# learnedsystems/RMI

Hardware: AMD Instinct MI355X
Metric: keys/s trained (200M uint64, linear,linear 1048576 leaves) (higher is better)
Workload: dtype f64

## Files before the change

### rmi_amd/csrc/rmi_hip.hip

```cpp
#include <hip/hip_runtime.h>

#include <algorithm>
#include <atomic>
#include <cstdarg>
#include <cstdio>
#include <cstdlib>
#include <cstring>
#include <cmath>
#include <functional>
#include <mutex>
#include <string>
#include <thread>
#include <vector>

#include "../../include/rmi_hip.h"
#include "rmi_kernels.hip.h"
#include "rmi_stream.hip.h"
#include "rmi_sigma.hip.h"
#include "rmi_lanes.hip.h"
#include "rmi_regs.hip.h"
#include "rmi_scan_launch.h"
#include "rmi_lookup_launch.h"
#include "rmi_root_host.h"
#include "rmi_route.h"
// ... 40 lines not shown
  rmi_route::Route last_route;
  bool tail_armed = false;
  std::function<int()> tail_fn;
  std::function<int(unsigned int)> regs_listed_fn;
  std::function<void()> refinalize_fn;
  unsigned int* d_tickets = nullptr;
  int peer_fuse_n = 0;
  unsigned char* peer_fuse_tab[7] = {};
  bool rows_pushed = false;
  hipEvent_t ev_stage[2] = {nullptr, nullptr};
  hipEvent_t ev[10] = {};
  int profile_level = 0;
  DevState* h_state_dev = nullptr;
  double* d_lntab = nullptr;
  double* d_regtab = nullptr;
  unsigned long long* d_regprof = nullptr;
  std::vector<rmi_hip_ctx*> many_views;
  void* d_bnext = nullptr; uint64_t bnext_cap = 0;
  unsigned char* d_tile_slow = nullptr; uint64_t tile_slow_cap = 0;
  unsigned int* d_slow_list = nullptr; uint64_t slow_cap = 0;
  int n_cu = 256;
  void* d_gaps = nullptr;
  unsigned int* d_tile_list = nullptr; uint64_t tile_list_cap = 0;
  bool lean_derived = false;
  unsigned long long lean_last_target = ~0ull, lean_leaf_lo = 0;
  uint64_t edge_first = 0, edge_last = 0, edge_epoch = 0, edgef_epoch = 0; double edge_first_f = 0.0, edge_last_f = 0.0;
  GiantLeaf* d_giant = nullptr; uint64_t giant_cap = 0;
  bool giant_armed = false;
  static constexpr uint64_t GIANT_EARLY_MAX = 256;
  unsigned long long* h_giant = nullptr;
// ... 84 lines not shown
  return RMI_OK;
}

extern "C" {

int rmi_hip_abi_version(void) { return RMI_HIP_ABI_VERSION; }
int rmi_hip_last_pipeline(rmi_hip_ctx* c) { return !c ? RMI_ERR_BAD_ARG : c->last_route.pipeline; }
int rmi_hip_last_route_info(rmi_hip_ctx* c, rmi_hip_route_info* out) {
  if (!c || !out || !c->last_L || !c->h_state) return RMI_ERR_BAD_ARG;
  const rmi_route::Route& r = c->last_route;
  const DevState& st = *c->h_state;
  std::memset(out, 0, sizeof *out);
  out->pipeline = r.pipeline; out->regs = r.regs;
  out->search = r.search; out->verify = r.verify; out->cubic_margin = r.cubic_margin; out->sigma = r.sigma;
  out->scan_mono = r.scan_mono; out->long_leaves = r.long_leaves; out->giants = r.giants;
  out->regs_listed = st.regs_listed; out->scan_listed = st.scan_listed; out->long_count = st.long_count; out->giant_count = st.giant_count;
  out->flag_count = st.flag_count; out->merged_count = st.merged_count; out->seg_count = st.seg_count; out->regs_dups = st.regs_dups;
  return RMI_OK;
}

int rmi_hip_device_count(void) {
  int n = 0;
  if (hipGetDeviceCount(&n) != hipSuccess) return 0;
  return n;
}

const char* rmi_hip_strerror(int code) {
  switch (code) {
    case RMI_OK: return "ok";
    case RMI_ERR_UNKNOWN_MODEL: return "unknown model type (train/mod.rs:53)";
// ... 82 lines not shown
  if (hipStreamCreateWithFlags(&c->own_stream, hipStreamNonBlocking) != hipSuccess) { rmi_hip_destroy(c); return RMI_ERR_HIP; }
  c->stream = c->own_stream;
  if (hipMalloc(&c->d_state, sizeof(DevState)) != hipSuccess) { rmi_hip_destroy(c); return RMI_ERR_HIP; }
  if (hipHostMalloc((void**)&c->h_state, sizeof(DevState) * RMI_STREAM_MAX_CHUNKS, hipHostMallocDefault) != hipSuccess ||
      hipHostGetDevicePointer((void**)&c->h_state_dev, c->h_state, 0) != hipSuccess) { rmi_hip_destroy(c); return RMI_ERR_HIP; }
  if (hipHostMalloc((void**)&c->h_sentinel, 64, hipHostMallocDefault) != hipSuccess) { rmi_hip_destroy(c); return RMI_ERR_HIP; }
  for (auto& e : c->ev) if (hipEventCreate(&e) != hipSuccess) { rmi_hip_destroy(c); return RMI_ERR_HIP; }
  c->profile_level = 0;
  c->knobs = rmi_route::read_knobs();
  { int cu = 0; if (hipDeviceGetAttribute(&cu, hipDeviceAttributeMultiprocessorCount, device_id) == hipSuccess && cu > 0) c->n_cu = cu; }
  if (hipMalloc(&c->d_lntab, sizeof(double) * (3 * LN_TMAX + 2 * (LS_SAMPLES + 1))) != hipSuccess) { rmi_hip_destroy(c); return RMI_ERR_HIP; }
  hipLaunchKernelGGL(k_lane_table, dim3((LN_TMAX + 255) / 256), dim3(256), 0, c->stream, c->d_lntab, LN_TMAX);
  if (hipMalloc(&c->d_regtab, sizeof(double) * 4 * RG_TMAX) != hipSuccess) { rmi_hip_destroy(c); return RMI_ERR_HIP; }
  if (RG_PROF) { if (hipMalloc(&c->d_regprof, 128) != hipSuccess || hipMemset(c->d_regprof, 0, 128) != hipSuccess) { rmi_hip_destroy(c); return RMI_ERR_HIP; } }
  hipLaunchKernelGGL(k_regs_table, dim3((RG_TMAX + 255) / 256), dim3(256), 0, c->stream, c->d_regtab, RG_TMAX);
  if (hipGetLastError() != hipSuccess || hipStreamSynchronize(c->stream) != hipSuccess) { rmi_hip_destroy(c); return RMI_ERR_HIP; }
  *out = c;
  return RMI_OK;
}

static void free_outputs(rmi_hip_ctx* c) {
  (void)hipFree(c->d_leaf_start); (void)hipFree(c->d_params); (void)hipFree(c->d_maxerr); (void)hipFree(c->d_run);
  (void)hipFree(c->d_err); (void)hipFree(c->d_count); (void)hipFree(c->d_rows); (void)hipFree(c->d_tilemin);
  (void)hipFree(c->d_partials); c->d_partials = nullptr;
  (void)hipFree(c->d_tickets); c->d_tickets = nullptr;
  release(c->d_long, c->long_cap); release(c->d_cube, c->cube_cap); release(c->d_flist, c->flist_cap); release(c->d_tile_list, c->tile_list_cap);
  release(c->d_bkeys, c->bkeys_cap); release(c->d_recs, c->recs_bytes); release(c->d_segs, c->segs_cap);
  if (c->d_flist_cnt) { (void)hipFree(c->d_flist_cnt); c->d_flist_cnt = nullptr; }
  if (c->d_gaps) { (void)hipFree(c->d_gaps); c->d_gaps = nullptr; }
  c->d_leaf_start = nullptr; c->d_params = nullptr; c->d_maxerr = nullptr; c->d_run = nullptr;
// ... 6 lines not shown
  if (!c) return;
  for (rmi_hip_ctx* v : c->many_views) rmi_hip_destroy(v);
  c->many_views.clear();
  for (rmi_hip_index* ix : c->indexes) index_release(ix);
  c->indexes.clear();
  if (c->upload_thread.joinable()) c->upload_thread.join();
  (void)hipSetDevice(c->device);
  if (c->stream) (void)hipStreamSynchronize(c->stream);
  free_multi(c);
  free_outputs(c);
  if (c->d_table) (void)hipFree(c->d_table);
  if (c->d_keys_owned) (void)hipFree(c->d_keys_owned);
  if (c->d_state) (void)hipFree(c->d_state);
  if (c->d_lntab) (void)hipFree(c->d_lntab);
  if (c->d_regtab) (void)hipFree(c->d_regtab);
  if (c->d_regprof) {
    unsigned long long h[16] = {};
    if (hipMemcpy(h, c->d_regprof, 128, hipMemcpyDeviceToHost) == hipSuccess)
      std::fprintf(stderr, "k_leaf_regs cycles (sum over waves and trainings): fit %llu, epilogue+tail %llu, hand-over %llu, error pass %llu, finalize %llu; (unused %llu) hand-over requests %llu, (unused %llu), finalize stores %llu, finalize up to the shuffles' end %llu; RG_PROF 2, inside the fit: panel requests %llu, stash %llu, arithmetic %llu, constants + landed %llu, wait for the panel %llu\n", h[0], h[1], h[2], h[3], h[4], h[5], h[6], h[7], h[8], h[9], h[5], h[7], h[8], h[9], h[11]);
    (void)hipFree(c->d_regprof);
  }
  release(c->d_slow_list, c->slow_cap); release(c->d_tile_slow, c->tile_slow_cap); release(c->d_bnext, c->bnext_cap); release(c->d_giant, c->giant_cap);
  if (c->h_state) (void)hipHostFree(c->h_state);
  if (c->h_sentinel) (void)hipHostFree(c->h_sentinel);
  for (int b = 0; b < 2; b++) { if (c->h_stage[b]) (void)hipHostFree(c->h_stage[b]); if (c->ev_stage[b]) (void)hipEventDestroy(c->ev_stage[b]); }
  if (c->copy_stream) (void)hipStreamDestroy(c->copy_stream);
  if (c->h_giant) (void)hipHostFree(c->h_giant);
  if (c->ev_giant) (void)hipEventDestroy(c->ev_giant);
  for (auto& e : c->ev) if (e) (void)hipEventDestroy(e);
  if (c->own_stream) (void)hipStreamDestroy(c->own_stream);
// ... 653 lines not shown

static inline uint64_t agg_records(uint64_t leaves) { const uint64_t w = (leaves + 63) / 64, m = (uint64_t)SCAN_MAX_WAVES + SCAN_GAP_BLOCKS; return w > m ? w : m; }
static inline uint64_t lane_slices(uint64_t leaves) { return (agg_records(leaves) + LF_SLICE - 1) / LF_SLICE; }
static int ensure_outputs(rmi_hip_ctx* c, uint64_t L, int ppl) {
  if (L <= c->cap_leaves && ppl <= c->cap_ppl) return RMI_OK;
  free_outputs(c);
  HIPCHK(c, hipMalloc(&c->d_leaf_start, (L + 1) * 8));
  HIPCHK(c, hipMalloc(&c->d_params, L * ppl * 8));
  HIPCHK(c, hipMalloc(&c->d_maxerr, L * 8));
  HIPCHK(c, hipMalloc(&c->d_run, L * 8));
  HIPCHK(c, hipMalloc(&c->d_err, L * 8));
  HIPCHK(c, hipMalloc(&c->d_count, L * 8));
  HIPCHK(c, hipMalloc(&c->d_rows, L * (ppl * 8 + 8)));
  HIPCHK(c, hipMalloc(&c->d_tilemin, ((L + 1 + FILL_TILE - 1) / FILL_TILE + 1) * 8));
  HIPCHK(c, hipMalloc(&c->d_partials, sizeof(StatsPartial) * (agg_records(L) + SG_REGIONS + 2 * FL_BLOCKS + 1 + lane_slices(L) + 1)));
  HIPCHK(c, hipMalloc(&c->d_tickets, 64));
  c->cap_leaves = L; c->cap_ppl = ppl;
  return RMI_OK;
}

static void host_cubes(double* v, uint64_t n) {
  unsigned nt = std::thread::hardware_concurrency();
  nt = nt < 1 ? 1 : (nt > 16 ? 16 : nt);
  if (n < 65536) nt = 1;
  auto work = [v](uint64_t a, uint64_t b) { for (uint64_t i = a; i < b; i++) v[i] = std::pow(v[i], 3.0); };
  if (nt == 1) { work(0, n); return; }
  std::vector<std::thread> th;
  const uint64_t per = (n + nt - 1) / nt;
  for (unsigned t = 0; t < nt; t++) {
    const uint64_t a = (uint64_t)t * per, b = a + per < n ? a + per : n;
    if (a < b) th.emplace_back(work, a, b);
// ... 90 lines not shown
    }
    if (r.giants_early) (void)launch_giant_list(c, a, fl);
    hipLaunchKernelGGL((k_list<K, LEAF>), dim3(128 * SG_REGIONS), dim3(64), 0, a.s, a.keys, a.sp, a.leaf_start, c->d_state, a.params, fl, sgp, a.maxerr, a.run,
                       dgiant, hmin, !r.giants_early);
    mk();
    hipLaunchKernelGGL((k_list_tail<K>), dim3(2048), dim3(64), 0, a.s, a.keys, a.sp, a.leaf_start, c->d_state, a.params, fl, c->d_segs, a.maxerr, a.run,
                       r.fused ? (const StatsPartial*)part : (const StatsPartial*)nullptr, (unsigned int)nrec, part + nrec);
    mk();
    if (r.fused)
      hipLaunchKernelGGL((k_finalize_listed<K>), dim3(FL_BLOCKS), dim3(FL_THREADS), 0, a.s, a.keys, a.sp, a.L, a.leaf_start, c->d_state, a.params, a.maxerr, a.run, a.err,
                         a.count, a.rows, fl, part + nrec, (unsigned int)SG_REGIONS, part + nrec + SG_REGIONS, c->d_flist_cnt + 2 * SG_REGIONS, c->d_state, hcopy,
                         (const GiantLeaf*)nullptr, hmin);
  };
  if (r.optimistic) {
    const unsigned int nsl = (unsigned int)((nrec + LF_SLICE - 1) / LF_SLICE);
    hipLaunchKernelGGL(k_lane_reduce, dim3(nsl), dim3(LF_SLICE), 0, a.s, (const StatsPartial*)part, (unsigned int)nrec, part + nrec + SG_REGIONS + 2 * FL_BLOCKS + 1,
                       c->d_tickets, fl, c->d_state, hcopy);
    a.mark(); a.mark();
    c->tail_armed = true;
    c->giant_early = r.giants_early;
    c->tail_fn = [tail]() -> int { tail([]() {}); return RMI_OK; };
  } else tail(a.mark);
}

template <typename K>
static int launch_regs(rmi_hip_ctx* c, const rmi_route::Route& r, const RootP& rp, Launch<K>& a, const SgList& fl, const PeerRows& peers) {
  const uint64_t wb = (a.L_own + 63) / 64;
  if (const int grc = grow(c, c->d_slow_list, c->slow_cap, wb, 4)) return grc;
  if (const int grc = grow(c, c->d_tile_slow, c->tile_slow_cap, wb, 1)) return grc;
  if (const int grc = grow(c, c->d_bnext, c->bnext_cap, wb, 64 * 16)) return grc;
  HIPCHK(c, hipGetLastError());
  const unsigned int lmin = lanes_long_min(c);
// ... 9 lines not shown
  else if constexpr (sizeof(K) == 4) regs(std::integral_constant<int, 2>{});
  a.mark();
  auto listed = [=](unsigned int grid_l) {
    hipLaunchKernelGGL((k_leaf_lanes_listed<K>), dim3(grid_l), dim3(64), 0, a.s, c->d_slow_list, c->d_tickets + 1, a.keys, a.sp, a.leaf_start, c->d_state, a.params,
                       c->d_lntab, fl, lmin, a.maxerr, a.run, a.L, a.err, a.count, a.rows, part, rp, peers);
  };
  if (r.listed_late) {
    const unsigned int wb_l = (unsigned int)wb;
    c->regs_listed_fn = [=](unsigned int groups) -> int {
      listed(groups < wb_l ? (groups > 0u ? groups : 1u) : wb_l);
      hipLaunchKernelGGL(k_lane_reduce, dim3((wb_l + LF_SLICE - 1) / LF_SLICE), dim3(LF_SLICE), 0, a.s, (const StatsPartial*)part, wb_l,
                         part + wb + SG_REGIONS + 2 * FL_BLOCKS + 1, c->d_tickets, fl, c->d_state, c->h_state_dev);
      return RMI_OK;
    };
  } else listed(wb < 512 ? (unsigned int)wb : 512u);
  auto finalize = [&](auto vroot, double scale) {
    hipLaunchKernelGGL((k_regs_finalize<K, decltype(vroot)::value>), dim3((unsigned)((wb * 64 + 255) / 256)), dim3(256), 0, a.s, a.keys, a.sp, a.L, a.leaf_start, c->d_state,
                       (const unsigned int*)(c->d_tickets + 1), a.params, (const unsigned long long*)a.maxerr, (const K*)bnext, (const K*)bprev,
                       (const unsigned char*)c->d_tile_slow, (unsigned int)wb, a.err, a.count, a.rows, part, peers, rp, scale, r.listed_late);
  };
  if (r.cubic_margin) finalize(std::integral_constant<int, K_CUBIC>{}, c->knobs.cubic_margin_scale);
  else finalize(std::integral_constant<int, -1>{}, 1.0);
  HIPCHK(c, hipGetLastError());
  return RMI_OK;
}

template <int ROOT, typename K>
static int launch_leaf_lanes(rmi_hip_ctx* c, const rmi_route::Route& r, const RootP& rp, Launch<K>& a) {
  hipStream_t s = a.s;
  const uint64_t L_own = a.L_own, wb = (L_own + 63) / 64;
  if (const int lrc = ensure_lists(c, a.n_it, L_own)) return lrc;
  if constexpr (ROOT == K_LINEAR || ROOT == K_RADIX || ROOT == K_CUBIC) {
    if (r.search) {
      const uint64_t sb = (L_own + (uint64_t)LS_BLOCK * LS_ILP - 1) / ((uint64_t)LS_BLOCK * LS_ILP);
      double* smp = c->d_lntab + 3 * LN_TMAX;
      LaneInit li; std::memset(&li, 0, sizeof li);
      if (r.init_folded) {
        li.st = c->d_state; li.init = a.init; li.leaf_start = a.a_leaf_start; li.L_own = L_own; li.sentinel = (unsigned long long)a.sp.it_hi;
        li.list_cnt = c->d_flist_cnt; li.n_list_cnt = 2 * SG_REGIONS + 8; li.tickets = c->d_tickets; li.n_tickets = 3;
      }
      hipLaunchKernelGGL((k_leaf_samples<ROOT, K>), dim3((LS_SAMPLES + 256) / 256), dim3(256), 0, s, a.keys, a.sp, rp, smp, li);
      hipLaunchKernelGGL((k_leaf_search<ROOT, K, LS_ILP>), dim3((unsigned)sb), dim3(LS_BLOCK), 0, s, a.keys, a.sp, rp, a.leaf_start, c->d_state, (const double*)smp);
    }
  }
  if (!r.init_folded) HIPCHK(c, hipMemsetAsync(c->d_tickets, 0, 12, s));
  if (!r.search) {
    launch_bounds<ROOT, K>(s, a.keys, a.n_it, a.sp, rp, a.leaf_start, c->d_state);
    launch_fill(s, a.a_leaf_start, L_own + 1, c->d_tilemin);
  }
  HIPCHK(c, a.mark.begin());
  const SgList fl = flist_of(c);
  if (r.giants) { if (const int grc = arm_giants(c, a)) return grc; }
  const PeerRows peers = peer_rows(c, r);
  auto lanes = [&](auto fused, auto vroot) {
// ... 556 lines not shown
```

### rmi_amd/csrc/rmi_lanes.hip.h

```cpp
#pragma once
#include <type_traits>

#include "rmi_device.hip.h"
#include "rmi_kernels.hip.h"
#include "rmi_stream.hip.h"
#include "rmi_sigma.hip.h"

#ifndef RMI_LN_NT_FIT
#define RMI_LN_NT_FIT 0
#endif
#ifndef RMI_LN_NT_ERR
#define RMI_LN_NT_ERR 1
#endif
#ifndef RMI_LN_WPE
#define RMI_LN_WPE 2
#endif
#ifndef RMI_LN_NBUF
#define RMI_LN_NBUF 2
#endif

namespace rmi {

template <typename K> struct LnGeom {
  static constexpr int KPL = 16 / (int)sizeof(K);
// ... 26 lines not shown

template <int ROOT, typename K>
__device__ __forceinline__ double ls_root_value(const RootP& r, K k) {
  if constexpr (ROOT == K_RADIX) {
    const uint64_t v = KeyTraits<K>::as_uint(k) << (r.prefix & 63u);
    return ldexp(KeyTraits<uint64_t>::as_float(v), -(int)((64u - r.bits) & 63u));
  } else return root_eval_f<ROOT>(r, KeyTraits<K>::as_float(k));
}

constexpr int LS_SAMPLES = 1024;
__device__ __forceinline__ uint64_t ls_sample_index(uint64_t A, uint64_t Bn, int t) {
  const uint64_t stride = (Bn - A - 1) / (uint64_t)LS_SAMPLES > 0 ? (Bn - A - 1) / (uint64_t)LS_SAMPLES : 1;
  const uint64_t i = A + (uint64_t)t * stride;
  return (t >= LS_SAMPLES || i >= Bn) ? Bn - 1 : i;
}
struct LaneInit {
  DevState* st; DevState init;
  unsigned long long* leaf_start; uint64_t L_own; unsigned long long sentinel;
  unsigned long long* list_cnt; int n_list_cnt;
  unsigned int* tickets; unsigned int n_tickets;
};
template <int ROOT, typename K>
__global__ void __launch_bounds__(256) k_leaf_samples(const K* __restrict__ keys, Span sp, RootP r, double* __restrict__ smp, LaneInit li) {
  const int t = blockIdx.x * 256 + threadIdx.x;
  if (li.st != nullptr && blockIdx.x == gridDim.x - 1) {
    for (int q = threadIdx.x; q < li.n_list_cnt; q += 256) li.list_cnt[q] = 0ull;
    for (unsigned int q = threadIdx.x; q < li.n_tickets; q += 256u) li.tickets[q] = 0u;
    if (threadIdx.x == 0) { *li.st = li.init; li.leaf_start[li.L_own] = li.sentinel; }
  }
  if (t > LS_SAMPLES || !(sp.it_hi > sp.it_lo)) return;
  const K k = keys[ls_sample_index(sp.it_lo, sp.it_hi, t)];
  bool oob;
  smp[t] = root_target_f<ROOT, K>(r, (double)(r.L - 1), k, oob);
  smp[LS_SAMPLES + 1 + t] = ls_root_value<ROOT, K>(r, k);
}

template <int ROOT, typename K, int ILP>
__global__ void __launch_bounds__(LS_BLOCK) k_leaf_search(const K* __restrict__ keys, Span sp, RootP r,
                                                          unsigned long long* __restrict__ leaf_start,
                                                          DevState* __restrict__ st, const double* __restrict__ smp) {
  typedef typename LnBits<K>::type BT;
  typedef BT vec_t __attribute__((ext_vector_type(2), aligned(sizeof(K))));
// ... 560 lines not shown
  if (!s_last) return;
  StatsPartial b{0ull, 0ull, 0ull, 0.0, 0.0};
  for (unsigned int t = threadIdx.x; t < gridDim.x; t += LF_SLICE) lf_combine(b, lf_load(slices + t));
  lf_block_reduce(b, &s_w);
  unsigned long long fc = threadIdx.x < (unsigned int)SG_REGIONS ? fl.cnt[threadIdx.x] : 0ull;
#pragma unroll
  for (int d = 32; d > 0; d >>= 1) fc += shfl_down_u64(fc, d);
  if (threadIdx.x == 0) {
    *ticket = 0u;
    st->max_err = b.mx; st->max_err_idx = b.mi; st->sum_n_err = b.sum; st->sum_l2 = b.l2; st->sum_log2 = b.lg;
    st->flag_count = fc; st->merged_count = 0; st->pending = fc;
    *host_copy = *st;
  }
}

constexpr int FL_BLOCKS = 1;
constexpr int FL_THREADS = 256;
template <typename K>
__global__ void __launch_bounds__(FL_THREADS) k_finalize_listed(const K* __restrict__ keys, Span sp, uint64_t L,
                                                         const unsigned long long* __restrict__ leaf_start,
                                                         const DevState* __restrict__ st, double* __restrict__ params,
                                                         const unsigned long long* __restrict__ leaf_maxerr,
                                                         const unsigned long long* __restrict__ leaf_run,
                                                         unsigned long long* __restrict__ leaf_err,
                                                         unsigned long long* __restrict__ leaf_count,
                                                         unsigned char* __restrict__ rows, SgList fl,
                                                         const StatsPartial* __restrict__ wave_partials, unsigned int nwave,
                                                         StatsPartial* __restrict__ out, unsigned long long* __restrict__ ticket,
                                                         DevState* __restrict__ stw, DevState* __restrict__ host_copy,
                                                         const GiantLeaf* __restrict__ flat, unsigned long long host_min) {
// ... 100 lines not shown
```

### rmi_amd/csrc/rmi_regs.hip.h

```cpp
#pragma once
#include <type_traits>

#include "rmi_lanes.hip.h"

namespace rmi {

#ifndef RG_STASH_N
#define RG_STASH_N 192
#endif
constexpr int RG_ROW = 16;
constexpr int RG_RING = 4;
constexpr int RG_PANEL_B = 64 * RG_ROW * 8;
constexpr int RG_STASH = RG_STASH_N;
#ifndef RG_STASH2_N
#define RG_STASH2_N 160
#endif
constexpr int RG_STASH2 = RG_STASH2_N;
constexpr int RG_MAXPTS = RG_STASH_N + 48;
constexpr int RG_FARPTS = 1008;
constexpr int RG_NBLK = RG_MAXPTS / RG_ROW;
constexpr int RG_SBLK = RG_STASH / RG_ROW;
static_assert(RG_NBLK - RG_SBLK <= RG_RING - 1, "the tail of a group must still be in the ring when its fit ends");
static_assert(RG_FARPTS + 16 <= 1024, "the step table (RG_TMAX) covers the walk");

// ... 633 lines not shown
    have = true;
    done_tile = tile;
    tile = tile2;
    tile2 = (unsigned int)__builtin_amdgcn_readfirstlane((int)tile3);
  }
  if (RG_PROF && prof != nullptr && lane == 0) {
#pragma unroll
    for (int i = 0; i < 12; i++) atomicAdd(prof + i, pf[i]);
  }
}

__device__ __forceinline__ uint64_t rg_readlane_u64(uint64_t v, int src) {
  const unsigned int lo = (unsigned int)__builtin_amdgcn_readlane((int)(unsigned int)v, src), hi = (unsigned int)__builtin_amdgcn_readlane((int)(unsigned int)(v >> 32), src);
  return ((uint64_t)hi << 32) | lo;
}
template <typename K, int VROOT = -1>
__global__ void __launch_bounds__(256) k_regs_finalize(const K* __restrict__ keys, Span sp, uint64_t L,
                                                       const unsigned long long* __restrict__ leaf_start, DevState* st, const unsigned int* __restrict__ slow_count,
                                                       double* __restrict__ params, const unsigned long long* __restrict__ leaf_maxerr,
                                                       const K* __restrict__ bnext, const K* __restrict__ bprev,
                                                       const unsigned char* __restrict__ tile_slow, unsigned int ntiles,
                                                       unsigned long long* __restrict__ leaf_err, unsigned long long* __restrict__ leaf_count,
                                                       unsigned char* __restrict__ rows, StatsPartial* __restrict__ partials, PeerRows peers, RootP vr,
                                                       double margin_scale,
                                                       bool listed_behind) {
  const uint64_t jl = (uint64_t)blockIdx.x * 256 + threadIdx.x;
  const unsigned int tile = (unsigned int)(jl >> 6);
  if (jl == 0) st->regs_listed = *slow_count;
  if (tile >= ntiles) return;
  const uint64_t j = sp.leaf_lo + jl;
  if constexpr (VROOT == K_CUBIC) {
    bool ok = true;
    uint64_t vs = 0, ve = 0;
    if (j < sp.leaf_hi) {
      const uint64_t s = leaf_start[j], e = leaf_start[j + 1];
      vs = s; ve = e;
      if (s < e) {
        auto val = [&](K k) -> double {
          const double x = KeyTraits<K>::as_float(k);
          const double v1 = __builtin_fma(vr.p0, x, vr.p1), v2 = __builtin_fma(v1, x, vr.p2), v3 = __builtin_fma(v2, x, vr.p3);
          return v3;
        };
        const uint64_t nl = sp.leaf_hi - sp.leaf_lo;
// ... 14 lines not shown
    const unsigned int Lm1 = (unsigned int)(vr.L - 1);
    while (um) {
      const int src = __builtin_ctzll(um);
      um &= um - 1ull;
      const uint64_t us = rg_readlane_u64(vs, src), ue = rg_readlane_u64(ve, src);
      const unsigned int uj = (unsigned int)(sp.leaf_lo + (jl & ~63ull) + (uint64_t)src);
      for (uint64_t i = us + (threadIdx.x & 63); i < ue; i += 64) {
        const unsigned int rt = sg_cvt_u32(root_eval_f<K_CUBIC>(vr, KeyTraits<K>::as_float(keys[i])));
        if (rt > Lm1) vflags |= EF_ROOT_OOB;
        if ((rt < Lm1 ? rt : Lm1) != uj) vflags |= EF_NON_MONOTONE;
      }
    }
    if (vflags) atomicOr(&st->err_flags, vflags);
  }
  if (tile_slow[tile] != 0) {
    if (listed_behind && (threadIdx.x & 63) == 0) partials[tile] = StatsPartial{0ull, 0ull, 0ull, 0.0, 0.0};
    return;
  }
  unsigned long long st_mx = 0, st_mi = 0, st_sum = 0;
  double st_l2 = 0.0, st_lg = 0.0;
  unsigned long long me = 0ull;
  uint64_t fs = 0, fe = 0;
  double fa = 0.0, fb = 0.0;
  if (j < sp.leaf_hi) { me = leaf_maxerr[j]; fs = leaf_start[j]; fe = leaf_start[j + 1]; fa = params[2 * j]; fb = params[2 * j + 1]; }
  {
    unsigned long long um = __ballot((me >> 63) != 0ull);
    const unsigned int n32 = (unsigned int)sp.n;
    const int ln = (int)(threadIdx.x & 63);
    while (um) {
      const int src = __builtin_ctzll(um);
      um &= um - 1ull;
// ... 5 lines not shown
        const double f = __builtin_fma(ub, KeyTraits<K>::as_float(keys[i]), ua);
        em = max(em, sg_absdiff(min(sg_cvt_u32(f), n32), (unsigned int)i));
      }
      em = rg_wave_max(em);
      if (ln == src) me = (unsigned long long)em;
    }
  }
  if (j < sp.leaf_hi) {
    const uint64_t s = fs, e = fe;
    double pp[2] = {fa, fb};
    const K k_next = e < sp.n ? bnext[jl] : KeyTraits<K>::max_value();
    const K k_prev = s > 0 ? bprev[jl] : KeyTraits<K>::zero_value();
    uint64_t final_err, cnt_j;
    finalize_one_pre<K_LINEAR, K>(j, s, e, sp, L, keys, pp, me, 0ull, st->last_target, k_next, k_prev, final_err, cnt_j);
    if (!(s < e)) { params[2 * j] = pp[0]; params[2 * j + 1] = pp[1]; }
    leaf_err[j] = final_err;
    leaf_count[j] = cnt_j;
    double* rp = reinterpret_cast<double*>(rows + j * 24);
    rp[0] = pp[0]; rp[1] = pp[1];
    *reinterpret_cast<unsigned long long*>(rows + j * 24 + 16) = final_err;
    for (int p = 0; p < peers.n; p++) {
      double* pr = reinterpret_cast<double*>(peers.tab[p] + j * 24);
      pr[0] = pp[0]; pr[1] = pp[1];
      *reinterpret_cast<unsigned long long*>(peers.tab[p] + j * 24 + 16) = final_err;
    }
    st_mx = final_err; st_mi = j;
    st_sum = cnt_j * final_err;
    const double v = (double)st_sum;
    st_l2 = (v * v) / (double)sp.n;
    st_lg = (double)cnt_j * log2((double)(2 * final_err + 2));
  }
#pragma unroll
  for (int d = 32; d > 0; d >>= 1) {
    const unsigned long long omx = shfl_down_u64(st_mx, d), omi = shfl_down_u64(st_mi, d);
    if (omx > st_mx || (omx == st_mx && omi > st_mi)) { st_mx = omx; st_mi = omi; }
    st_sum += shfl_down_u64(st_sum, d);
    st_l2 += __shfl_down(st_l2, d);
    st_lg += __shfl_down(st_lg, d);
  }
  if ((threadIdx.x & 63) == 0) partials[tile] = StatsPartial{st_mx, st_mi, st_sum, st_l2, st_lg};
}

template <typename K>
__global__ void __launch_bounds__(64) __attribute__((amdgpu_waves_per_eu(RMI_LN_WPE, RMI_LN_WPE))) k_leaf_lanes_listed(const unsigned int* __restrict__ slow_list,
                                                   const unsigned int* __restrict__ slow_count, const K* __restrict__ keys, Span sp,
                                                   const unsigned long long* __restrict__ leaf_start,
                                                   DevState* __restrict__ st, double* __restrict__ params,
                                                   const double* __restrict__ rtab, SgList fl, unsigned int long_min,
                                                   unsigned long long* __restrict__ leaf_maxerr,
                                                   unsigned long long* __restrict__ leaf_run, uint64_t L,
                                                   unsigned long long* __restrict__ leaf_err,
                                                   unsigned long long* __restrict__ leaf_count,
                                                   unsigned char* __restrict__ rows, StatsPartial* __restrict__ partials, RootP vr,
                                                   PeerRows peers) {
  __shared__ typename LnBits<K>::type panel[64 * LnGeom<K>::STRIDE];
// ... 8 lines not shown
```

### rmi_amd/csrc/rmi_route.h

```cpp
#pragma once

#include <algorithm>
#include <cstdint>
#include <cstdlib>
#include <functional>

#include "../../include/rmi_hip.h"

namespace rmi_route {

constexpr uint64_t IDX32_LIMIT = (1ull << 32) - (1ull << 16);
constexpr uint64_t SIGMA_MIN_LEAF = 32;
constexpr uint64_t SCAN_SKEW_LISTED = 512;

struct Knobs {
  int pipeline = 3;
  bool lanes_search = true;
  bool opt_tail = true;
  uint64_t host_min = 262144;
  bool host_min_set = false;
  bool regs = true;
  bool regs_forced = false;
  int regs_u32 = 2;
  unsigned int regs_grid = 0;
  unsigned int regs_max_avg = 208;
  unsigned int regs_long_max_avg = 640;
  bool regs_backoff = true;
  bool cubic_margin = true;
  double cubic_margin_scale = 1.0;
  bool lean = true;
  unsigned int scan_waves = 0;
  uint64_t fit_threads = 131072;
  int fit_min_chunk = 64;
  unsigned int long_min = 4096;
};

inline Knobs read_knobs() {
  Knobs k;
  auto env = [](const char* name) -> const char* { const char* v = std::getenv(name); return v && *v ? v : nullptr; };
  if (const char* v = env("RMI_HIP_PIPELINE")) k.pipeline = std::atoi(v) >= 3 ? 3 : 2;
  if (const char* v = env("RMI_HIP_LANES_SEARCH")) k.lanes_search = std::atoi(v) != 0;
  if (const char* v = env("RMI_HIP_OPT_TAIL")) k.opt_tail = std::atoi(v) != 0;
  if (const char* v = env("RMI_HIP_HOST_MIN")) { k.host_min = std::strtoull(v, nullptr, 10); k.host_min_set = true; }
  if (const char* v = env("RMI_HIP_REGS")) { k.regs = std::atoi(v) != 0; k.regs_forced = k.regs; }
  if (const char* v = env("RMI_HIP_REGS_U32")) k.regs_u32 = std::atoi(v);
  if (const char* v = env("RMI_HIP_REGS_GRID")) k.regs_grid = (unsigned int)std::atoi(v);
  if (const char* v = env("RMI_HIP_REGS_MAX_AVG")) k.regs_max_avg = (unsigned int)std::atoi(v);
  if (const char* v = env("RMI_HIP_REGS_LONG_MAX_AVG")) k.regs_long_max_avg = (unsigned int)std::atoi(v);
  if (const char* v = env("RMI_HIP_REGS_BACKOFF")) k.regs_backoff = std::atoi(v) != 0;
  if (const char* v = env("RMI_HIP_CUBIC_MARGIN")) k.cubic_margin = std::atoi(v) != 0;
  if (const char* v = env("RMI_HIP_CUBIC_MARGIN_SCALE")) k.cubic_margin_scale = std::atof(v);
  if (const char* v = env("RMI_HIP_LEAN")) k.lean = std::atoi(v) != 0;
  if (const char* v = env("RMI_HIP_SCAN_WAVES")) k.scan_waves = (unsigned int)std::atoi(v);
  if (const char* v = env("RMI_HIP_FIT_THREADS")) k.fit_threads = std::strtoull(v, nullptr, 10);
  if (const char* v = env("RMI_HIP_FIT_MIN_CHUNK")) k.fit_min_chunk = std::atoi(v);
  if (const char* v = env("RMI_HIP_LONG_MIN")) { const long l = std::atol(v); if (l >= 64) k.long_min = (unsigned int)l; }
  return k;
// ... 16 lines not shown

struct Route {
  int pipeline = 2;
  bool sigma = false;
  bool search = false;
  bool init_folded = false;
  bool fused = false;
  bool optimistic = false;
  bool listed_late = false;
  bool peers = false;
  bool giants = false, giants_early = false;
  int regs = -1;
  unsigned int regs_grid = 0;
  bool verify = false;
  bool cubic_margin = false;
  bool scan_mono = false, lean = false, long_leaves = false;
  unsigned int listed_hint = ~0u;
  bool lanes() const { return pipeline >= 3; }
  bool init_arrays() const { return pipeline != 5 && !init_folded; }
};

inline Route plan_route(const Knobs& k, const RouteIn& in) {
  Route r;
  const bool idx32 = in.n < IDX32_LIMIT, u32 = in.key_type == RMI_KEY_U32;
  const bool linear_leaf = in.leaf_kind == RMI_MODEL_LINEAR;
  const bool linear_root = in.root_kind == RMI_MODEL_LINEAR || in.root_kind == RMI_MODEL_ROBUST_LINEAR || in.root_kind == RMI_MODEL_LINEAR_SPLINE;
  const bool radix_root = in.root_kind == RMI_MODEL_RADIX || in.root_kind == RMI_MODEL_BRADIX, cubic_root = in.root_kind == RMI_MODEL_CUBIC;
  const uint64_t L = in.L_own;
  const bool scan = k.pipeline >= 3 && in.leaf_kind == RMI_MODEL_LINEAR_SPLINE && idx32;
  r.sigma = linear_leaf && in.fit_mode != 0 && !in.sigma_hinted && idx32 && in.n_it >= SIGMA_MIN_LEAF * L && in.n_it >= 4096;
// ... 20 lines not shown
  }
  r.pipeline = 3;
  const uint64_t wb = (L + 63) / 64, resident = 4ull * (uint64_t)in.n_cu;
  const bool regs_long = in.n_it > (uint64_t)k.regs_max_avg * L;
  const unsigned int cap = k.regs_long_max_avg > k.regs_max_avg ? k.regs_long_max_avg : k.regs_max_avg;
  bool regs = r.fused && k.regs && !in.regs_off && in.n_it <= (uint64_t)cap * L && (!u32 || k.regs_u32);
  if (!regs_long && !k.regs_forced && k.regs_grid == 0 && wb > resident && 2 * wb <= 5 * resident) regs = false;
  if (cubic_root && linear_leaf && r.search && regs && k.cubic_margin) r.cubic_margin = in.cubic_increasing();
  r.verify = cubic_root && linear_leaf && r.search && !r.cubic_margin;
  if (regs && !r.verify) {
    r.pipeline = 4;
    const bool w2 = u32 && k.regs_u32 >= 2;
    r.regs = w2 ? 2 : regs_long ? 1 : 0;
    const uint64_t grid = k.regs_grid ? k.regs_grid : (w2 ? 8ull : 4ull) * (uint64_t)in.n_cu;
    r.regs_grid = (unsigned int)(grid > wb ? wb : grid);
  }
  return r;
}

struct RouteKey { uint64_t epoch; uint64_t L_own; int fit_mode; };
struct TrainCounts { uint64_t scan_listed, flag_count, merged_count; unsigned int regs_listed; };
struct RouteMemory {
  uint64_t hint_epoch = 0, hint_L[8] = {};
  int hint_n = 0, hint_mode = -1;
  uint64_t regs_off_epoch = 0, regs_off_L[8] = {};
  int regs_off_n = 0;
  uint64_t scan_hint_epoch = 0, scan_hint_L = 0; unsigned int scan_hint_n = ~0u;
  uint64_t scan_skew_epoch = ~0ull, scan_skew_L = 0;

  void lookup(const RouteKey& key, RouteIn* in) const {
// ... 24 lines not shown
```

### rmi_amd/train.py

```python
from __future__ import annotations

import ctypes as C
import re
import threading
import time
from dataclasses import dataclass, field

import numpy as np

from . import _lib

KEY_U64, KEY_U32, KEY_F64 = 0, 1, 2
_DTYPES = {np.dtype(np.uint64): KEY_U64, np.dtype(np.uint32): KEY_U32, np.dtype(np.float64): KEY_F64}

MODEL_NAMES = ["linear", "linear_spline", "cubic", "radix", "robust_linear", "loglinear", "normal",
               "lognormal", "radix8", "radix18", "radix22", "radix26", "radix28", "bradix", "histogram"]


class RMIError(RuntimeError):

    def __init__(self, code: int, detail: str = ""):
        lib = _lib.load()
        msg = lib.rmi_hip_strerror(code).decode()
        super().__init__(f"rmi_hip error {code}: {msg}" + (f" [{detail}]" if detail else ""))
# ... 316 lines not shown
            device_ns=int(res.device_ns), kernel_ns=tuple(res.kernel_ns), long_leaves=int(res.long_leaves),
            split_idx=int(res.split_idx), split_target=int(res.split_target),
            shard_leaf_lo=int(res.shard_leaf_lo), shard_leaves=int(res.shard_leaves),
            partial={"max_error": int(res.model_max_error), "max_error_idx": int(res.model_max_error_idx),
                     "sum_n_err": int(res.sum_n_err), "sum_l2": float(res.sum_l2), "sum_log2": float(res.sum_log2)},
            fit_mode_used=int(res.fit_mode_used), exact_leaves=int(res.exact_leaves), merged_leaves=int(res.merged_leaves), guard_leaves=int(res.guard_leaves),
            generation=int(res.generation), pipeline=int(self._lib.rmi_hip_last_pipeline(self._h)), _trainer=self)

    def last_route(self):
        fn = getattr(self._lib, "rmi_hip_last_route_info", None)
        info = _lib.RouteInfo()
        with self._ctx_lock:
            if fn is None or self._h is None or fn(self._h, C.byref(info)) != 0:
                return None
        flags = ("search", "verify", "cubic_margin", "sigma", "scan_mono", "long_leaves", "giants")
        return {n: (bool(getattr(info, n)) if n in flags else int(getattr(info, n))) for n, _ in _lib.RouteInfo._fields_ if not n.startswith("_")}

    def train_many(self, configs, in_flight: int = 4):
        self.wait_keys()
        n = len(configs)
        cfg = (_lib.TrainConfig * max(n, 1))()
        kinds, keep = [], []
        for i, (root, leaf, L) in enumerate(configs):
            lk = leaf if isinstance(leaf, int) else MODEL_NAMES.index(leaf)
            kinds.append(lk)
            cfg[i].root = root._c()
            cfg[i].leaf_kind = lk
            cfg[i].num_leaves = int(L)
            if root.is_radix_table:
                if root.table is None:
                    raise ValueError("a radix-table root needs its hint table (Model.table)")
# ... 142 lines not shown
```

Measured before the change: 427.0 billion.

## Fuse lane stats reduction into regs finalize via last-block tickets

Removes the separate k_lane_reduce launch by having k_regs_finalize blocks count arrivals per slice with atomics. The last block of each slice reduces the slice, and the last slice publishes the global stats to device and host state. It also replaces the per-leaf log2 with a precomputed table for small errors, swaps the final four shuffle rounds for DPP row shifts, and in lean mode skips the per-leaf err/count writes. The cost is extra atomics and a tail serialisation in the last blocks, plus more complex ticket reset logic.

```diff
diff --git a/rmi_amd/csrc/rmi_hip.hip b/rmi_amd/csrc/rmi_hip.hip
--- a/rmi_amd/csrc/rmi_hip.hip
+++ b/rmi_amd/csrc/rmi_hip.hip
@@ -78,6 +78,7 @@
   DevState* h_state_dev = nullptr;
   double* d_lntab = nullptr;
   double* d_regtab = nullptr;
+  double* d_l2tab = nullptr;
   unsigned long long* d_regprof = nullptr;
   std::vector<rmi_hip_ctx*> many_views;
   void* d_bnext = nullptr; uint64_t bnext_cap = 0;
@@ -192,6 +193,7 @@
   out->pipeline = r.pipeline; out->regs = r.regs;
   out->search = r.search; out->verify = r.verify; out->cubic_margin = r.cubic_margin; out->sigma = r.sigma;
   out->scan_mono = r.scan_mono; out->long_leaves = r.long_leaves; out->giants = r.giants;
+  out->_pad = (r.tail_fused ? 1 : 0) | (r.lean ? 2 : 0);
   out->regs_listed = st.regs_listed; out->scan_listed = st.scan_listed; out->long_count = st.long_count; out->giant_count = st.giant_count;
   out->flag_count = st.flag_count; out->merged_count = st.merged_count; out->seg_count = st.seg_count; out->regs_dups = st.regs_dups;
   return RMI_OK;
@@ -304,6 +306,8 @@
   if (hipMalloc(&c->d_regtab, sizeof(double) * 4 * RG_TMAX) != hipSuccess) { rmi_hip_destroy(c); return RMI_ERR_HIP; }
   if (RG_PROF) { if (hipMalloc(&c->d_regprof, 128) != hipSuccess || hipMemset(c->d_regprof, 0, 128) != hipSuccess) { rmi_hip_destroy(c); return RMI_ERR_HIP; } }
   hipLaunchKernelGGL(k_regs_table, dim3((RG_TMAX + 255) / 256), dim3(256), 0, c->stream, c->d_regtab, RG_TMAX);
+  if (hipMalloc(&c->d_l2tab, sizeof(double) * RG_L2TAB) != hipSuccess) { rmi_hip_destroy(c); return RMI_ERR_HIP; }
+  hipLaunchKernelGGL(k_regs_log2_table, dim3((RG_L2TAB + 255) / 256), dim3(256), 0, c->stream, c->d_l2tab, RG_L2TAB);
   if (hipGetLastError() != hipSuccess || hipStreamSynchronize(c->stream) != hipSuccess) { rmi_hip_destroy(c); return RMI_ERR_HIP; }
   *out = c;
   return RMI_OK;
@@ -340,6 +344,7 @@
   if (c->d_state) (void)hipFree(c->d_state);
   if (c->d_lntab) (void)hipFree(c->d_lntab);
   if (c->d_regtab) (void)hipFree(c->d_regtab);
+  if (c->d_l2tab) (void)hipFree(c->d_l2tab);
   if (c->d_regprof) {
     unsigned long long h[16] = {};
     if (hipMemcpy(h, c->d_regprof, 128, hipMemcpyDeviceToHost) == hipSuccess)
@@ -1023,7 +1028,7 @@
   HIPCHK(c, hipMalloc(&c->d_rows, L * (ppl * 8 + 8)));
   HIPCHK(c, hipMalloc(&c->d_tilemin, ((L + 1 + FILL_TILE - 1) / FILL_TILE + 1) * 8));
   HIPCHK(c, hipMalloc(&c->d_partials, sizeof(StatsPartial) * (agg_records(L) + SG_REGIONS + 2 * FL_BLOCKS + 1 + lane_slices(L) + 1)));
-  HIPCHK(c, hipMalloc(&c->d_tickets, 64));
+  HIPCHK(c, hipMalloc(&c->d_tickets, 4 * lf_ticket_words(lane_slices(L))));
   c->cap_leaves = L; c->cap_ppl = ppl;
   return RMI_OK;
 }
@@ -1144,8 +1149,9 @@
   };
   if (r.optimistic) {
     const unsigned int nsl = (unsigned int)((nrec + LF_SLICE - 1) / LF_SLICE);
-    hipLaunchKernelGGL(k_lane_reduce, dim3(nsl), dim3(LF_SLICE), 0, a.s, (const StatsPartial*)part, (unsigned int)nrec, part + nrec + SG_REGIONS + 2 * FL_BLOCKS + 1,
-                       c->d_tickets, fl, c->d_state, hcopy);
+    if (!r.tail_fused)
+      hipLaunchKernelGGL(k_lane_reduce, dim3(nsl), dim3(LF_SLICE), 0, a.s, (const StatsPartial*)part, (unsigned int)nrec, part + nrec + SG_REGIONS + 2 * FL_BLOCKS + 1,
+                         c->d_tickets, fl, c->d_state, hcopy);
     a.mark(); a.mark();
     c->tail_armed = true;
     c->giant_early = r.giants_early;
@@ -1185,13 +1191,19 @@
       return RMI_OK;
     };
   } else listed(wb < 512 ? (unsigned int)wb : 512u);
-  auto finalize = [&](auto vroot, double scale) {
-    hipLaunchKernelGGL((k_regs_finalize<K, decltype(vroot)::value>), dim3((unsigned)((wb * 64 + 255) / 256)), dim3(256), 0, a.s, a.keys, a.sp, a.L, a.leaf_start, c->d_state,
-                       (const unsigned int*)(c->d_tickets + 1), a.params, (const unsigned long long*)a.maxerr, (const K*)bnext, (const K*)bprev,
-                       (const unsigned char*)c->d_tile_slow, (unsigned int)wb, a.err, a.count, a.rows, part, peers, rp, scale, r.listed_late);
+  LaneTail lt; std::memset(&lt, 0, sizeof lt);
+  lt.slices = part + wb + SG_REGIONS + 2 * FL_BLOCKS + 1; lt.tickets = c->d_tickets; lt.fl = fl; lt.host_copy = c->h_state_dev;
+  auto finalize = [&](auto vroot, auto fused, double scale) {
+    hipLaunchKernelGGL((k_regs_finalize<K, decltype(vroot)::value, decltype(fused)::value>), dim3((unsigned)((wb * 64 + 255) / 256)), dim3(256), 0, a.s, a.keys, a.sp, a.L,
+                       a.leaf_start, c->d_state, (const unsigned int*)(c->d_tickets + 1), a.params, (const unsigned long long*)a.maxerr, (const K*)bnext, (const K*)bprev,
+                       (const unsigned char*)c->d_tile_slow, (unsigned int)wb, r.lean ? nullptr : a.err, r.lean ? nullptr : a.count, a.rows, part, peers, rp, scale, r.listed_late,
+                       lt, (const double*)c->d_l2tab);
   };
-  if (r.cubic_margin) finalize(std::integral_constant<int, K_CUBIC>{}, c->knobs.cubic_margin_scale);
-  else finalize(std::integral_constant<int, -1>{}, 1.0);
+  auto finalize_root = [&](auto fused) {
+    if (r.cubic_margin) finalize(std::integral_constant<int, K_CUBIC>{}, fused, c->knobs.cubic_margin_scale);
+    else finalize(std::integral_constant<int, -1>{}, fused, 1.0);
+  };
+  if (r.tail_fused) finalize_root(std::true_type{}); else finalize_root(std::false_type{});
   HIPCHK(c, hipGetLastError());
   return RMI_OK;
 }
@@ -1209,6 +1221,7 @@
       if (r.init_folded) {
         li.st = c->d_state; li.init = a.init; li.leaf_start = a.a_leaf_start; li.L_own = L_own; li.sentinel = (unsigned long long)a.sp.it_hi;
         li.list_cnt = c->d_flist_cnt; li.n_list_cnt = 2 * SG_REGIONS + 8; li.tickets = c->d_tickets; li.n_tickets = 3;
+        li.n_slice_cnt = r.tail_fused ? (unsigned int)((wb + LF_SLICE - 1) / LF_SLICE) : 0u;
       }
       hipLaunchKernelGGL((k_leaf_samples<ROOT, K>), dim3((LS_SAMPLES + 256) / 256), dim3(256), 0, s, a.keys, a.sp, rp, smp, li);
       hipLaunchKernelGGL((k_leaf_search<ROOT, K, LS_ILP>), dim3((unsigned)sb), dim3(LS_BLOCK), 0, s, a.keys, a.sp, rp, a.leaf_start, c->d_state, (const double*)smp);
diff --git a/rmi_amd/csrc/rmi_lanes.hip.h b/rmi_amd/csrc/rmi_lanes.hip.h
--- a/rmi_amd/csrc/rmi_lanes.hip.h
+++ b/rmi_amd/csrc/rmi_lanes.hip.h
@@ -64,11 +64,13 @@
   const uint64_t i = A + (uint64_t)t * stride;
   return (t >= LS_SAMPLES || i >= Bn) ? Bn - 1 : i;
 }
+constexpr unsigned int LF_CNT_BASE = 16, LF_CNT_STRIDE = 16;
 struct LaneInit {
   DevState* st; DevState init;
   unsigned long long* leaf_start; uint64_t L_own; unsigned long long sentinel;
   unsigned long long* list_cnt; int n_list_cnt;
   unsigned int* tickets; unsigned int n_tickets;
+  unsigned int n_slice_cnt;
 };
 template <int ROOT, typename K>
 __global__ void __launch_bounds__(256) k_leaf_samples(const K* __restrict__ keys, Span sp, RootP r, double* __restrict__ smp, LaneInit li) {
@@ -76,6 +78,7 @@
   if (li.st != nullptr && blockIdx.x == gridDim.x - 1) {
     for (int q = threadIdx.x; q < li.n_list_cnt; q += 256) li.list_cnt[q] = 0ull;
     for (unsigned int q = threadIdx.x; q < li.n_tickets; q += 256u) li.tickets[q] = 0u;
+    for (unsigned int q = threadIdx.x; q < li.n_slice_cnt; q += 256u) li.tickets[LF_CNT_BASE + q * LF_CNT_STRIDE] = 0u;
     if (threadIdx.x == 0) { *li.st = li.init; li.leaf_start[li.L_own] = li.sentinel; }
   }
   if (t > LS_SAMPLES || !(sp.it_hi > sp.it_lo)) return;
@@ -666,6 +669,56 @@
   }
 }
 
+static inline uint64_t lf_ticket_words(uint64_t slices) { return LF_CNT_BASE + slices * LF_CNT_STRIDE; }
+struct LaneTail {
+  StatsPartial* slices; unsigned int* tickets; SgList fl; DevState* host_copy;
+};
+template <bool OWN_FLAGS>
+__device__ __forceinline__ void lf_arrive_publish(const StatsPartial* partials, unsigned int nrec, const LaneTail& lt, DevState* st, unsigned int regs_listed) {
+  static_assert(LF_SLICE == 128 && SG_REGIONS == 64, "32 blocks of four records a slice; one hand-over counter per lane");
+  constexpr unsigned int BPS = LF_SLICE / 4;
+  __shared__ StatsPartial s_w;
+  __shared__ bool s_last;
+  const unsigned int slice = blockIdx.x / BPS, nsl = (nrec + LF_SLICE - 1) / LF_SLICE;
+  unsigned int* const cnt = lt.tickets + LF_CNT_BASE + slice * LF_CNT_STRIDE;
+  asm volatile("s_waitcnt vmcnt(0)" ::: "memory");
+  __syncthreads();
+  if (threadIdx.x == 0) {
+    const unsigned int left = gridDim.x - slice * BPS, expect = left < BPS ? left : BPS;
+    s_last = __hip_atomic_fetch_add(cnt, 1u, __ATOMIC_RELAXED, __HIP_MEMORY_SCOPE_AGENT) == expect - 1u;
+  }
+  __syncthreads();
+  if (!s_last) return;
+  const unsigned int q = slice * LF_SLICE + threadIdx.x;
+  StatsPartial a{0ull, 0ull, 0ull, 0.0, 0.0};
+  if (threadIdx.x < LF_SLICE && q < nrec) a = lf_load(partials + q);
+  lf_block_reduce(a, &s_w);
+  if (threadIdx.x == 0) {
+    lf_store(lt.slices + slice, a);
+    __hip_atomic_store(cnt, 0u, __ATOMIC_RELAXED, __HIP_MEMORY_SCOPE_AGENT);
+    s_last = __hip_atomic_fetch_add(lt.tickets, 1u, __ATOMIC_RELAXED, __HIP_MEMORY_SCOPE_AGENT) == nsl - 1u;
+  }
+  __syncthreads();
+  if (!s_last) return;
+  StatsPartial b{0ull, 0ull, 0ull, 0.0, 0.0};
+  if (threadIdx.x < LF_SLICE)
+    for (unsigned int t = threadIdx.x; t < nsl; t += LF_SLICE) lf_combine(b, lf_load(lt.slices + t));
+  lf_block_reduce(b, &s_w);
+  unsigned long long fc = threadIdx.x < (unsigned int)SG_REGIONS ? lt.fl.cnt[threadIdx.x] : 0ull;
+#pragma unroll
+  for (int d = 32; d > 0; d >>= 1) fc += shfl_down_u64(fc, d);
+  if (threadIdx.x == 0) {
+    __hip_atomic_store(lt.tickets, 0u, __ATOMIC_RELAXED, __HIP_MEMORY_SCOPE_AGENT);
+    if constexpr (OWN_FLAGS) {
+      st->err_flags = __hip_atomic_fetch_or((volatile unsigned int*)&st->err_flags, 0u, __ATOMIC_RELAXED, __HIP_MEMORY_SCOPE_AGENT);
+    }
+    st->regs_listed = regs_listed;
+    st->max_err = b.mx; st->max_err_idx = b.mi; st->sum_n_err = b.sum; st->sum_l2 = b.l2; st->sum_log2 = b.lg;
+    st->flag_count = fc; st->merged_count = 0; st->pending = fc;
+    *lt.host_copy = *st;
+  }
+}
+
 constexpr int FL_BLOCKS = 1;
 constexpr int FL_THREADS = 256;
 template <typename K>
diff --git a/rmi_amd/csrc/rmi_regs.hip.h b/rmi_amd/csrc/rmi_regs.hip.h
--- a/rmi_amd/csrc/rmi_regs.hip.h
+++ b/rmi_amd/csrc/rmi_regs.hip.h
@@ -671,8 +671,22 @@
   const unsigned int lo = (unsigned int)__builtin_amdgcn_readlane((int)(unsigned int)v, src), hi = (unsigned int)__builtin_amdgcn_readlane((int)(unsigned int)(v >> 32), src);
   return ((uint64_t)hi << 32) | lo;
 }
-template <typename K, int VROOT = -1>
-__global__ void __launch_bounds__(256) k_regs_finalize(const K* __restrict__ keys, Span sp, uint64_t L,
+constexpr int RG_L2TAB = 4096;
+static __global__ void __launch_bounds__(256) k_regs_log2_table(double* __restrict__ tab, int count) {
+  const int e = blockIdx.x * blockDim.x + threadIdx.x;
+  if (e < count) tab[e] = log2((double)(2ull * (unsigned long long)e + 2ull));
+}
+template <int D> __device__ __forceinline__ unsigned long long rg_row_down_u64(unsigned long long v) {
+  const unsigned int lo = (unsigned int)v, hi = (unsigned int)(v >> 32);
+  const unsigned int ol = (unsigned int)__builtin_amdgcn_update_dpp((int)lo, (int)lo, 0x100 + D, 0xF, 0xF, false);
+  const unsigned int oh = (unsigned int)__builtin_amdgcn_update_dpp((int)hi, (int)hi, 0x100 + D, 0xF, 0xF, false);
+  return ((unsigned long long)oh << 32) | ol;
+}
+template <int D> __device__ __forceinline__ double rg_row_down_f64(double v) {
+  return __longlong_as_double((long long)rg_row_down_u64<D>((unsigned long long)__double_as_longlong(v)));
+}
+template <typename K, int VROOT, bool FUSED>
+__device__ __forceinline__ void regs_finalize_leaves(const K* __restrict__ keys, Span sp, uint64_t L,
                                                        const unsigned long long* __restrict__ leaf_start, DevState* st, const unsigned int* __restrict__ slow_count,
                                                        double* __restrict__ params, const unsigned long long* __restrict__ leaf_maxerr,
                                                        const K* __restrict__ bnext, const K* __restrict__ bprev,
@@ -680,10 +694,10 @@
                                                        unsigned long long* __restrict__ leaf_err, unsigned long long* __restrict__ leaf_count,
                                                        unsigned char* __restrict__ rows, StatsPartial* __restrict__ partials, PeerRows peers, RootP vr,
                                                        double margin_scale,
-                                                       bool listed_behind) {
+                                                       bool listed_behind, const double* __restrict__ l2tab) {
   const uint64_t jl = (uint64_t)blockIdx.x * 256 + threadIdx.x;
   const unsigned int tile = (unsigned int)(jl >> 6);
-  if (jl == 0) st->regs_listed = *slow_count;
+  if (!FUSED && jl == 0) st->regs_listed = *slow_count;
   if (tile >= ntiles) return;
   const uint64_t j = sp.leaf_lo + jl;
   if constexpr (VROOT == K_CUBIC) {
@@ -728,7 +742,10 @@
     if (vflags) atomicOr(&st->err_flags, vflags);
   }
   if (tile_slow[tile] != 0) {
-    if (listed_behind && (threadIdx.x & 63) == 0) partials[tile] = StatsPartial{0ull, 0ull, 0ull, 0.0, 0.0};
+    if (listed_behind && (threadIdx.x & 63) == 0) {
+      const StatsPartial none{0ull, 0ull, 0ull, 0.0, 0.0};
+      if constexpr (FUSED) lf_store(partials + tile, none); else partials[tile] = none;
+    }
     return;
   }
   unsigned long long st_mx = 0, st_mi = 0, st_sum = 0;
@@ -764,8 +781,7 @@
     uint64_t final_err, cnt_j;
     finalize_one_pre<K_LINEAR, K>(j, s, e, sp, L, keys, pp, me, 0ull, st->last_target, k_next, k_prev, final_err, cnt_j);
     if (!(s < e)) { params[2 * j] = pp[0]; params[2 * j + 1] = pp[1]; }
-    leaf_err[j] = final_err;
-    leaf_count[j] = cnt_j;
+    if (!FUSED || leaf_err != nullptr) { leaf_err[j] = final_err; leaf_count[j] = cnt_j; }
     double* rp = reinterpret_cast<double*>(rows + j * 24);
     rp[0] = pp[0]; rp[1] = pp[1];
     *reinterpret_cast<unsigned long long*>(rows + j * 24 + 16) = final_err;
@@ -778,17 +794,50 @@
     st_sum = cnt_j * final_err;
     const double v = (double)st_sum;
     st_l2 = (v * v) / (double)sp.n;
-    st_lg = (double)cnt_j * log2((double)(2 * final_err + 2));
-  }
-#pragma unroll
-  for (int d = 32; d > 0; d >>= 1) {
+    double lg;
+    if (FUSED && final_err < (uint64_t)RG_L2TAB) lg = l2tab[final_err];
+    else lg = log2((double)(2 * final_err + 2));
+    st_lg = (double)cnt_j * lg;
+  }
+#pragma unroll
+  for (int d = 32; d > (FUSED ? 8 : 0); d >>= 1) {
     const unsigned long long omx = shfl_down_u64(st_mx, d), omi = shfl_down_u64(st_mi, d);
     if (omx > st_mx || (omx == st_mx && omi > st_mi)) { st_mx = omx; st_mi = omi; }
     st_sum += shfl_down_u64(st_sum, d);
     st_l2 += __shfl_down(st_l2, d);
     st_lg += __shfl_down(st_lg, d);
   }
-  if ((threadIdx.x & 63) == 0) partials[tile] = StatsPartial{st_mx, st_mi, st_sum, st_l2, st_lg};
+  if constexpr (FUSED) {
+    auto round = [&](auto dtag) {
+      constexpr int D = decltype(dtag)::value;
+      const unsigned long long omx = rg_row_down_u64<D>(st_mx), omi = rg_row_down_u64<D>(st_mi);
+      const unsigned long long osum = rg_row_down_u64<D>(st_sum);
+      const double ol2 = rg_row_down_f64<D>(st_l2), olg = rg_row_down_f64<D>(st_lg);
+      if (omx > st_mx || (omx == st_mx && omi > st_mi)) { st_mx = omx; st_mi = omi; }
+      st_sum += osum; st_l2 += ol2; st_lg += olg;
+    };
+    round(std::integral_constant<int, 8>{}); round(std::integral_constant<int, 4>{});
+    round(std::integral_constant<int, 2>{}); round(std::integral_constant<int, 1>{});
+  }
+  if ((threadIdx.x & 63) == 0) {
+    const StatsPartial rec{st_mx, st_mi, st_sum, st_l2, st_lg};
+    if constexpr (FUSED) lf_store(partials + tile, rec); else partials[tile] = rec;
+  }
+}
+template <typename K, int VROOT = -1, bool FUSED = false>
+__global__ void __launch_bounds__(256) k_regs_finalize(const K* __restrict__ keys, Span sp, uint64_t L,
+                                                       const unsigned long long* __restrict__ leaf_start, DevState* st, const unsigned int* __restrict__ slow_count,
+                                                       double* __restrict__ params, const unsigned long long* __restrict__ leaf_maxerr,
+                                                       const K* __restrict__ bnext, const K* __restrict__ bprev,
+                                                       const unsigned char* __restrict__ tile_slow, unsigned int ntiles,
+                                                       unsigned long long* __restrict__ leaf_err, unsigned long long* __restrict__ leaf_count,
+                                                       unsigned char* __restrict__ rows, StatsPartial* __restrict__ partials, PeerRows peers, RootP vr,
+                                                       double margin_scale,
+                                                       bool listed_behind,
+                                                       LaneTail lt, const double* __restrict__ l2tab) {
+  regs_finalize_leaves<K, VROOT, FUSED>(keys, sp, L, leaf_start, st, slow_count, params, leaf_maxerr, bnext, bprev, tile_slow, ntiles, leaf_err, leaf_count, rows,
+                                        partials, peers, vr, margin_scale, listed_behind, l2tab);
+  if constexpr (FUSED) lf_arrive_publish<VROOT == K_CUBIC>(partials, ntiles, lt, st, *slow_count);
 }
 
 template <typename K>
diff --git a/rmi_amd/csrc/rmi_route.h b/rmi_amd/csrc/rmi_route.h
--- a/rmi_amd/csrc/rmi_route.h
+++ b/rmi_amd/csrc/rmi_route.h
@@ -17,6 +17,7 @@
   int pipeline = 3;
   bool lanes_search = true;
   bool opt_tail = true;
+  bool tail_fused = true;
   uint64_t host_min = 262144;
   bool host_min_set = false;
   bool regs = true;
@@ -41,6 +42,7 @@
   if (const char* v = env("RMI_HIP_PIPELINE")) k.pipeline = std::atoi(v) >= 3 ? 3 : 2;
   if (const char* v = env("RMI_HIP_LANES_SEARCH")) k.lanes_search = std::atoi(v) != 0;
   if (const char* v = env("RMI_HIP_OPT_TAIL")) k.opt_tail = std::atoi(v) != 0;
+  if (const char* v = env("RMI_HIP_TAIL_FUSED")) k.tail_fused = std::atoi(v) != 0;
   if (const char* v = env("RMI_HIP_HOST_MIN")) { k.host_min = std::strtoull(v, nullptr, 10); k.host_min_set = true; }
   if (const char* v = env("RMI_HIP_REGS")) { k.regs = std::atoi(v) != 0; k.regs_forced = k.regs; }
   if (const char* v = env("RMI_HIP_REGS_U32")) k.regs_u32 = std::atoi(v);
@@ -87,6 +89,7 @@
   unsigned int regs_grid = 0;
   bool verify = false;
   bool cubic_margin = false;
+  bool tail_fused = false;
   bool scan_mono = false, lean = false, long_leaves = false;
   unsigned int listed_hint = ~0u;
   bool lanes() const { return pipeline >= 3; }
@@ -137,6 +140,8 @@
     r.regs = w2 ? 2 : regs_long ? 1 : 0;
     const uint64_t grid = k.regs_grid ? k.regs_grid : (w2 ? 8ull : 4ull) * (uint64_t)in.n_cu;
     r.regs_grid = (unsigned int)(grid > wb ? wb : grid);
+    r.tail_fused = k.tail_fused && r.search && r.init_folded && r.optimistic && r.listed_late && !in.rows_ext;
+    r.lean = r.tail_fused && k.lean;
   }
   return r;
 }
diff --git a/rmi_amd/train.py b/rmi_amd/train.py
--- a/rmi_amd/train.py
+++ b/rmi_amd/train.py
@@ -354,7 +354,9 @@
             if fn is None or self._h is None or fn(self._h, C.byref(info)) != 0:
                 return None
         flags = ("search", "verify", "cubic_margin", "sigma", "scan_mono", "long_leaves", "giants")
-        return {n: (bool(getattr(info, n)) if n in flags else int(getattr(info, n))) for n, _ in _lib.RouteInfo._fields_ if not n.startswith("_")}
+        out = {n: (bool(getattr(info, n)) if n in flags else int(getattr(info, n))) for n, _ in _lib.RouteInfo._fields_ if not n.startswith("_")}
+        out["tail_fused"], out["lean"] = bool(info._pad & 1), bool(info._pad & 2)
+        return out
 
     def train_many(self, configs, in_flight: int = 4):
         self.wait_keys()
```

Measured after the change: 429.5 billion (median of 4 runs). Within noise of the previous version (+0.6%).
